# Ipsedo/MusicGAN

Hardware: AMD Instinct MI355X
Metric: spectrogram-images/sec G+D step, 2x128x128 bs64 (higher is better)
Workload: dtype f32

## Files before the change

musicgan_amd/csrc/wino_strip.hip:

```cpp
#include <cstdlib>
#include <type_traits>
#include <utility>

#include "mg_common.h"
#include "pack_kernels.h"
#include "wino_common.h"

namespace {

typedef float f32x2 __attribute__((ext_vector_type(2)));
typedef unsigned u32x2 __attribute__((ext_vector_type(2)));
typedef unsigned u32x4 __attribute__((ext_vector_type(4)));

enum StripKind {
  SK_ACT = 0,
  SK_ACT_POOL_MOUT,
  SK_MB_POOL,
  SK_MASKF,
  SK_UNPOOL,
  SK_BLEND_FWD,
  SK_BLEND_TAN,
  SK_BLEND_BWD,
  SK_PN,
  SK_MB_Y,
};

__device__ __forceinline__ unsigned f2u(float v) { return __builtin_bit_cast(unsigned, v); }
__device__ __forceinline__ int f2i(float v) { return __builtin_bit_cast(int, v); }
__device__ __forceinline__ int clamp01(int v) { return v < 0 ? 0 : (v > 1 ? 1 : v); }
__device__ __forceinline__ float sel_bits(int t, float x, float y) {
  return __builtin_bit_cast(float, (t & f2i(x)) | (~t & f2i(y)));
}

template <class F, int... Is>
__device__ __forceinline__ void sk_static_for_impl(F&& f, std::integer_sequence<int, Is...>) {
  (f(std::integral_constant<int, Is>{}), ...);
}
template <int N, class F>
__device__ __forceinline__ void sk_static_for(F&& f) {
  sk_static_for_impl(f, std::make_integer_sequence<int, N>{});
}
template <int OFF>
__device__ __forceinline__ f32x4 sk_lds128(unsigned addr) {
  f32x4 v;
  asm volatile("ds_read_b128 %0, %1 offset:%2" : "=v"(v) : "v"(addr), "n"(OFF));
  return v;
}
__device__ __forceinline__ void sk_wait() { asm volatile("s_waitcnt lgkmcnt(0)" ::: "memory"); }
__device__ __forceinline__ void sk_tie(f32x4& v) { asm volatile("" : "+v"(v)); }

template <int NIW, int NLDS, int NWAVE, int KIND, bool POOL>
__device__ __forceinline__ void strip_body(const WinoArgs& a, const int ct0, const int wg, const int G) {
  constexpr int kind = KIND;
  constexpr int NTHR = 64 * NWAVE;
  extern __shared__ __attribute__((aligned(16))) float smem[];
  float* Us = smem;
  const int tid = threadIdx.x;
  const int lane = tid & 63, col = lane & 15, rq = lane >> 4;
  const int wave = __builtin_amdgcn_readfirstlane(tid >> 6);
  const int HW = a.H * a.W;
  const int Ht = a.H >> 1, Wt = a.W >> 1;
  const int PP = Ht * Wt;

  {
    const int n4 = a.nchunk * NLDS * 512;
    const f32x4* src = reinterpret_cast<const f32x4*>(a.up);
    f32x4* dst = reinterpret_cast<f32x4*>(Us);
    for (int i = tid; i < n4; i += NTHR) {
      const int ch = i / (NLDS * 512), r = i - ch * (NLDS * 512);
      dst[i] = src[((size_t)ch * a.NT + ct0) * 512 + r];
    }
  }
  __syncthreads();

  const int groups_y = Ht / NWAVE;
  const int nitems = a.N * groups_y * a.blocks_x;
  const int first = mg_xcd_remap(wg, G);
  if (first >= nitems) return;
  const int dbx = G % a.blocks_x, dgy = (G / a.blocks_x) % groups_y, dn = G / (a.blocks_x * groups_y);
  int bx = first % a.blocks_x, gy = (first / a.blocks_x) % groups_y, n0 = first / (a.blocks_x * groups_y);
  int item = first;
  int by = gy * NWAVE + wave;
  auto step = [&](int& item_, int& bx_, int& gy_, int& n_) __attribute__((always_inline)) {
    item_ += G;
    bx_ += dbx;
    const int c1 = bx_ >= a.blocks_x ? 1 : 0;
    bx_ -= c1 * a.blocks_x;
    gy_ += dgy + c1;
    const int c2 = gy_ >= groups_y ? 1 : 0;
    gy_ -= c2 * groups_y;
    n_ += dn + c2;
  };
  auto advance = [&]() __attribute__((always_inline)) {
    step(item, bx, gy, n0);
    by = gy * NWAVE + wave;
  };

  const int lp = ((2 * rq) * HW + 2 * col) * 4;
  unsigned vP, vX;
  int rowoff[4];
  int rowrec[4];
  const float* img_base;
  auto block_geometry = [&]() __attribute__((always_inline)) {
    img_base = a.x + (size_t)n0 * a.Cin * HW;
    const int xoff = bx * 128;
    vP = (unsigned)(lp + xoff);
    vX = col == 0 ? (bx == 0 ? 0x80000000u : vP - 4u) : ((col == 15 && bx != a.blocks_x - 1) ? vP + 8u : 0x80000000u);
#pragma unroll
    for (int r = 0; r < 4; ++r) {
      const int Y = 2 * by - 1 + r;
      rowoff[r] = Y * a.W * 4;
      rowrec[r] = (item < nitems && Y >= 0 && Y < a.H && !(a.TBN & 2)) ? a.Cin * HW * 4 : 0;
    }
  };

  f32x4 acc[16][NIW];
  f32x2 rP[2][4];
  float rX[2][4];
  f32x2 V[2][8];

  auto load_rows = [&](int ch) __attribute__((always_inline)) {
#pragma unroll
    for (int r = 0; r < 4; ++r) {
      const __amdgpu_buffer_rsrc_t rsrc = __builtin_amdgcn_make_buffer_rsrc(const_cast<float*>(img_base), 0, rowrec[r], 0x00020000);
#pragma unroll
      for (int ks = 0; ks < 2; ++ks) {
        const int soff = (ch * WCC + ks) * HW * 4 + rowoff[r];
        rP[ks][r] = __builtin_bit_cast(f32x2, __builtin_amdgcn_raw_buffer_load_b64(rsrc, (int)vP, soff, 0));
        rX[ks][r] = __builtin_bit_cast(float, __builtin_amdgcn_raw_buffer_load_b32(rsrc, (int)vX, soff, 0));
      }
    }
  };

  auto transform_rows = [&]() __attribute__((always_inline)) {
#pragma unroll
    for (int ks = 0; ks < 2; ++ks) {
      f32x2 rE[4];
#pragma unroll
      for (int r = 0; r < 4; ++r) {
        const int old = __builtin_bit_cast(int, rX[ks][r]);
        rE[r][0] = __builtin_bit_cast(float, __builtin_amdgcn_update_dpp(old, __builtin_bit_cast(int, f2i(rP[ks][r][1])), 0x111, 0xf, 0xf, false));
        rE[r][1] = __builtin_bit_cast(float, __builtin_amdgcn_update_dpp(old, __builtin_bit_cast(int, f2i(rP[ks][r][0])), 0x101, 0xf, 0xf, false));
      }
      f32x2 UE[4], UP[4];
      UE[0] = pk_sub(rE[0], rE[2]);  UP[0] = pk_sub(rP[ks][0], rP[ks][2]);
      UE[1] = rE[1] + rE[2];         UP[1] = rP[ks][1] + rP[ks][2];
      UE[2] = pk_sub(rE[2], rE[1]);  UP[2] = pk_sub(rP[ks][2], rP[ks][1]);
      UE[3] = pk_sub(rE[1], rE[3]);  UP[3] = pk_sub(rP[ks][1], rP[ks][3]);
      asm("v_pk_add_f32 %0, %8, %12 op_sel:[0,1] op_sel_hi:[1,0] neg_lo:[0,1] neg_hi:[1,0]\n\t"
          "v_pk_add_f32 %1, %12, %12 op_sel:[0,1] op_sel_hi:[1,0] neg_lo:[0,0] neg_hi:[0,1]\n\t"
          "v_pk_add_f32 %2, %9, %13 op_sel:[0,1] op_sel_hi:[1,0] neg_lo:[0,1] neg_hi:[1,0]\n\t"
          "v_pk_add_f32 %3, %13, %13 op_sel:[0,1] op_sel_hi:[1,0] neg_lo:[0,0] neg_hi:[0,1]\n\t"
          "v_pk_add_f32 %4, %10, %14 op_sel:[0,1] op_sel_hi:[1,0] neg_lo:[0,1] neg_hi:[1,0]\n\t"
          "v_pk_add_f32 %5, %14, %14 op_sel:[0,1] op_sel_hi:[1,0] neg_lo:[0,0] neg_hi:[0,1]\n\t"
          "v_pk_add_f32 %6, %11, %15 op_sel:[0,1] op_sel_hi:[1,0] neg_lo:[0,1] neg_hi:[1,0]\n\t"
          "v_pk_add_f32 %7, %15, %15 op_sel:[0,1] op_sel_hi:[1,0] neg_lo:[0,0] neg_hi:[0,1]\n\t"
          "s_nop 1"
          : "=&v"(V[ks][0]), "=&v"(V[ks][1]), "=&v"(V[ks][2]), "=&v"(V[ks][3]), "=&v"(V[ks][4]), "=&v"(V[ks][5]), "=&v"(V[ks][6]), "=&v"(V[ks][7])
          : "v"(UE[0]), "v"(UE[1]), "v"(UE[2]), "v"(UE[3]), "v"(UP[0]), "v"(UP[1]), "v"(UP[2]), "v"(UP[3]));
    }
  };

  const unsigned us_lane = (unsigned)reinterpret_cast<size_t>(Us + lane * 4);
  auto mfma_chunk = [&](int ch, auto first_) __attribute__((always_inline)) {
    constexpr bool FIRST = decltype(first_)::value;
    const unsigned ub = us_lane + (unsigned)(ch * NLDS) * 8192u;
    f32x4 bv[2][NIW];
    sk_static_for<NIW>([&](auto ni_) __attribute__((always_inline)) {
      constexpr int ni = decltype(ni_)::value;
      bv[0][ni] = sk_lds128<ni * 8192>(ub);
    });
    sk_static_for<8>([&](auto cp_) __attribute__((always_inline)) {
      constexpr int cp = decltype(cp_)::value;
      constexpr int cur = cp & 1, nxt = cur ^ 1;
      sk_wait();
#pragma unroll
      for (int ni = 0; ni < NIW; ++ni) sk_tie(bv[cur][ni]);
      if constexpr (cp + 1 < 8) {
        sk_static_for<NIW>([&](auto ni_) __attribute__((always_inline)) {
          constexpr int ni = decltype(ni_)::value;
          bv[nxt][ni] = sk_lds128<ni * 8192 + (cp + 1) * 1024>(ub);
        });
      }
      __builtin_amdgcn_sched_barrier(0);
#pragma unroll
      for (int ks = 0; ks < 2; ++ks)
#pragma unroll
        for (int par = 0; par < 2; ++par)
#pragma unroll
          for (int ni = 0; ni < NIW; ++ni) {
            const f32x4 c0 = (FIRST && ks == 0) ? f32x4{0.f, 0.f, 0.f, 0.f} : acc[2 * cp + par][ni];
            acc[2 * cp + par][ni] = __builtin_amdgcn_mfma_f32_16x16x4f32(bv[cur][ni][ks * 2 + par], V[ks][cp][par], c0, 0, 0, 0);
          }
      __builtin_amdgcn_sched_barrier(0);
    });
  };

  const bool lrelu = (a.flags & MG_CONV_LRELU) != 0;
  const float slope = a.slope;
  const float slope_eff = lrelu ? slope : 1.0f;
  auto bias4 = [&](int ni) __attribute__((always_inline)) {
    f32x4 b = f32x4{0.f, 0.f, 0.f, 0.f};
    if (a.bias != nullptr) b = *reinterpret_cast<const f32x4*>(a.bias + (ct0 + ni) * 16 + rq * 4);
    return b;
  };
  auto xform = [&](int ni, f32x4 (&r4)[4]) __attribute__((always_inline)) {
    asm volatile("s_nop 7\n\ts_nop 7" : "+v"(acc[0][ni]), "+v"(acc[1][ni]), "+v"(acc[2][ni]), "+v"(acc[3][ni]), "+v"(acc[4][ni]),
                 "+v"(acc[5][ni]), "+v"(acc[6][ni]), "+v"(acc[7][ni]));
    asm volatile("" : "+v"(acc[8][ni]), "+v"(acc[9][ni]), "+v"(acc[10][ni]), "+v"(acc[11][ni]), "+v"(acc[12][ni]), "+v"(acc[13][ni]),
                 "+v"(acc[14][ni]), "+v"(acc[15][ni]));
    constexpr int SL[4] = {0, 2, 3, 1};
    f32x4 s0[4], s1[4];
#pragma unroll
    for (int nu = 0; nu < 4; ++nu) {
      const f32x4 m0 = acc[SL[nu]][ni], m1 = acc[4 + SL[nu]][ni], m2 = acc[8 + SL[nu]][ni], m3 = acc[12 + SL[nu]][ni];
      s0[nu] = (m0 + m1) + m2;
      s1[nu] = pk_sub4(pk_sub4(m1, m2), m3);
    }
    r4[0] = (s0[0] + s0[1]) + s0[2];
    r4[1] = pk_sub4(pk_sub4(s0[1], s0[2]), s0[3]);
    r4[2] = (s1[0] + s1[1]) + s1[2];
    r4[3] = pk_sub4(pk_sub4(s1[1], s1[2]), s1[3]);
  };
  auto activate = [&](int ni, f32x4 (&r4)[4]) __attribute__((always_inline)) {
    const f32x4 b4 = bias4(ni);
#pragma unroll
    for (int q = 0; q < 4; ++q) {
      const f32x4 v = r4[q] + b4;
      const f32x4 w = v * slope_eff;
#pragma unroll
      for (int g = 0; g < 4; ++g) r4[q][g] = fmaxf(v[g], w[g]);
    }
  };
  auto mask_bits = [&](const f32x4 (&r4)[4], int g) __attribute__((always_inline)) {
    const int b0 = clamp01(f2i(r4[0][g])), b1 = clamp01(f2i(r4[1][g])), b2 = clamp01(f2i(r4[2][g])), b3 = clamp01(f2i(r4[3][g]));
    return ((b0 | (b1 << 1)) | (b2 << 2)) | (b3 << 3);
  };
  auto apply_mask_bytes = [&](f32x4 (&r4)[4], const unsigned (&mb)[4]) __attribute__((always_inline)) {
#pragma unroll
    for (int q = 0; q < 4; ++q) {
      const f32x4 os = r4[q] * slope;
#pragma unroll
      for (int g = 0; g < 4; ++g) r4[q][g] = sel_bits(__builtin_amdgcn_sbfe((int)mb[g], q, 1), r4[q][g], os[g]);
    }
  };

  auto acc_fence = [&]() __attribute__((always_inline)) {};
  const int ly = ((rq * 4) * HW + 2 * col) * 4;
  const int lpo = ((rq * 4) * PP + col) * 4;
  using T_ = std::true_type;
  using F_ = std::false_type;

  const int nch = a.nchunk;
  block_geometry();
  load_rows(0);
  transform_rows();
#pragma nounroll
  for (;;) {
    const int ebx = bx, eby = by, en0 = n0;
    load_rows(1);
    mfma_chunk(0, T_{});
    for (int ch = 1; ch + 1 < nch; ++ch) {
      transform_rows();
      load_rows(ch + 1);
      mfma_chunk(ch, F_{});
    }
    transform_rows();
    advance();
    block_geometry();
    load_rows(0);
    mfma_chunk(nch - 1, F_{});
    __builtin_amdgcn_sched_barrier(0);
    acc_fence();
    transform_rows();
    __builtin_amdgcn_sched_barrier(0);

    {
      const int sy = ((2 * eby) * a.W + 32 * ebx) * 4;
      const int sp = (eby * Wt + 16 * ebx) * 4;
      const int yoff = ly, poff = lpo;
      const int TX = ebx * 16 + col;
      const int W4 = a.W * 4;
      auto rs = [&](const void* base, size_t img_elems, int esize) __attribute__((always_inline)) {
        return __builtin_amdgcn_make_buffer_rsrc(const_cast<char*>(reinterpret_cast<const char*>(base)) + (size_t)en0 * img_elems * esize,
                                                 0, (a.TBN & 4) ? 0 : (int)(img_elems * esize), 0x00020000);
      };
      const size_t full = (size_t)a.Cout * HW, pooled_n = (size_t)a.Cout * PP;
      auto store_rows = [&](__amdgpu_buffer_rsrc_t r, const f32x4 (&r4)[4], int ni) __attribute__((always_inline)) {
#pragma unroll
        for (int g4 = 0; g4 < 4; ++g4) {
          const int so = ((ct0 + ni) * 16 + g4) * HW * 4 + sy;
          __builtin_amdgcn_raw_buffer_store_b64(__builtin_bit_cast(u32x2, f32x2{r4[0][g4], r4[1][g4]}), r, yoff, so, 0);
          __builtin_amdgcn_raw_buffer_store_b64(__builtin_bit_cast(u32x2, f32x2{r4[2][g4], r4[3][g4]}), r, yoff, so + W4, 0);
        }
      };
      auto load_rows_f = [&](__amdgpu_buffer_rsrc_t r, f32x4 (&o4)[4], int ni) __attribute__((always_inline)) {
#pragma unroll
        for (int g4 = 0; g4 < 4; ++g4) {
          const int so = ((ct0 + ni) * 16 + g4) * HW * 4 + sy;
          const f32x2 t0 = __builtin_bit_cast(f32x2, __builtin_amdgcn_raw_buffer_load_b64(r, yoff, so, 0));
          const f32x2 t1 = __builtin_bit_cast(f32x2, __builtin_amdgcn_raw_buffer_load_b64(r, yoff, so + W4, 0));
          o4[0][g4] = t0[0]; o4[1][g4] = t0[1]; o4[2][g4] = t1[0]; o4[3][g4] = t1[1];
        }
      };
      auto store_pooled = [&](__amdgpu_buffer_rsrc_t r, const f32x4 (&r4)[4], int ni) __attribute__((always_inline)) {
        const f32x4 pl = ((r4[0] + r4[1]) + (r4[2] + r4[3])) * 0.25f;
#pragma unroll
        for (int g4 = 0; g4 < 4; ++g4)
          __builtin_amdgcn_raw_buffer_store_b32(f2u(pl[g4]), r, poff, ((ct0 + ni) * 16 + g4) * PP * 4 + sp, 0);
      };
      auto load_mask_bytes = [&](__amdgpu_buffer_rsrc_t r, unsigned (&mb)[4], int ni) __attribute__((always_inline)) {
#pragma unroll
        for (int g4 = 0; g4 < 4; ++g4) mb[g4] = __builtin_amdgcn_raw_buffer_load_b8(r, poff >> 2, ((ct0 + ni) * 16 + g4) * PP + (sp >> 2), 0);
      };
      auto store_mask_bytes = [&](__amdgpu_buffer_rsrc_t r, const f32x4 (&r4)[4], int ni) __attribute__((always_inline)) {
#pragma unroll
        for (int g4 = 0; g4 < 4; ++g4)
          __builtin_amdgcn_raw_buffer_store_b8((unsigned char)mask_bits(r4, g4), r, poff >> 2, ((ct0 + ni) * 16 + g4) * PP + (sp >> 2), 0);
      };
      constexpr bool act_on = false;

      if constexpr (kind == SK_ACT_POOL_MOUT) {
        const auto rp = rs(a.p, pooled_n, 4), rm = rs(a.mo, pooled_n, 1);
#pragma unroll
        for (int ni = 0; ni < NIW; ++ni) {
          f32x4 r4[4];
          xform(ni, r4);
          activate(ni, r4);
          store_mask_bytes(rm, r4, ni);
          store_pooled(rp, r4, ni);
        }
      } else if constexpr (kind == SK_MB_POOL) {
        const auto rp = rs(a.p, pooled_n, 4), rm = rs(a.mi, pooled_n, 1);
#pragma unroll
        for (int ni = 0; ni < NIW; ++ni) {
          unsigned mb[4];
          load_mask_bytes(rm, mb, ni);
          f32x4 r4[4];
          xform(ni, r4);
          if (act_on) activate(ni, r4);
          apply_mask_bytes(r4, mb);
          store_pooled(rp, r4, ni);
        }
      } else if constexpr (kind == SK_ACT) {
        const auto ry = rs(a.y, full, 4), rp = rs(a.p, pooled_n, 4);
#pragma unroll
        for (int ni = 0; ni < NIW; ++ni) {
          f32x4 r4[4];
          xform(ni, r4);
          activate(ni, r4);
          store_rows(ry, r4, ni);
          if (POOL) store_pooled(rp, r4, ni);
        }
      } else if constexpr (kind == SK_MASKF) {
        const auto ry = rs(a.y, full, 4), rx = rs(a.aux, full, 4), rp = rs(a.p, pooled_n, 4);
#pragma unroll
        for (int ni = 0; ni < NIW; ++ni) {
          f32x4 ax[4];
          load_rows_f(rx, ax, ni);
          f32x4 r4[4];
          xform(ni, r4);
          if (act_on) activate(ni, r4);
#pragma unroll
          for (int q = 0; q < 4; ++q) {
            const f32x4 os = r4[q] * slope;
#pragma unroll
            for (int g4 = 0; g4 < 4; ++g4) r4[q][g4] = ax[q][g4] > 0.f ? r4[q][g4] : os[g4];
          }
          store_rows(ry, r4, ni);
          if (POOL) store_pooled(rp, r4, ni);
        }
      } else if constexpr (kind == SK_UNPOOL) {
        const auto ry = rs(a.y, 4 * full, 4), rm = rs(a.aux, full, 1);
        const int uoff = yoff >> 2, su = sy >> 2;
        const int y2off = ((rq * 4) * 4 * HW + 4 * col) * 4;
        const int sy2 = ((4 * eby) * (2 * a.W) + 64 * ebx) * 4;
        const float qh = 0.25f, ql = 0.25f * slope;
#pragma unroll
        for (int ni = 0; ni < NIW; ++ni) {
          unsigned mw[4][2];
#pragma unroll
          for (int g4 = 0; g4 < 4; ++g4)
#pragma unroll
            for (int i = 0; i < 2; ++i)
              mw[g4][i] = __builtin_amdgcn_raw_buffer_load_b16(rm, uoff, ((ct0 + ni) * 16 + g4) * HW + i * a.W + su, 0);
          f32x4 r4[4];
          xform(ni, r4);
#pragma unroll
          for (int g4 = 0; g4 < 4; ++g4)
#pragma unroll
            for (int i = 0; i < 2; ++i) {
              const float vh[2] = {r4[2 * i][g4] * qh, r4[2 * i + 1][g4] * qh}, vl[2] = {r4[2 * i][g4] * ql, r4[2 * i + 1][g4] * ql};
#pragma unroll
              for (int r = 0; r < 2; ++r) {
                f32x4 o;
#pragma unroll
                for (int e = 0; e < 2; ++e)
#pragma unroll
                  for (int jj = 0; jj < 2; ++jj)
                    o[e * 2 + jj] = sel_bits(__builtin_amdgcn_sbfe((int)mw[g4][i], 8 * e + 2 * r + jj, 1), vh[e], vl[e]);
                __builtin_amdgcn_raw_buffer_store_b128(__builtin_bit_cast(u32x4, o), ry, y2off,
                                                       (((ct0 + ni) * 16 + g4) * 4 * HW + (2 * i + r) * 2 * a.W) * 4 + sy2, 0);
                asm volatile("s_nop 1" : "+v"(o) : : "memory");
              }
            }
        }
      } else if constexpr (kind == SK_BLEND_FWD || kind == SK_BLEND_TAN) {
        const auto ry = rs(a.y, full, 4), ro = rs(a.other, full, 4);
        const auto rm = rs(kind == SK_BLEND_FWD ? static_cast<const void*>(a.mo) : static_cast<const void*>(a.mi), pooled_n, 1);
        const float bca = a.coef[0], bcb = a.coef[1];
#pragma unroll
        for (int ni = 0; ni < NIW; ++ni) {
          f32x4 o4[4];
          load_rows_f(ro, o4, ni);
          unsigned mb[4] = {15u, 15u, 15u, 15u};
          if (kind == SK_BLEND_TAN) load_mask_bytes(rm, mb, ni);
          f32x4 r4[4];
          xform(ni, r4);
          if (kind == SK_BLEND_FWD || act_on) activate(ni, r4);
          if (kind == SK_BLEND_TAN) apply_mask_bytes(r4, mb);
          else store_mask_bytes(rm, r4, ni);
#pragma unroll
          for (int q = 0; q < 4; ++q) r4[q] = bca * r4[q] + bcb * o4[q];
          store_rows(ry, r4, ni);
        }
      } else if constexpr (kind == SK_BLEND_BWD) {
        const auto ry = rs(a.y, full, 4), rp = rs(a.p, full, 4), ro = rs(a.other, full, 4), rm = rs(a.mi, pooled_n, 1);
        const float ca = a.coef[0], cb = a.coef[1];
#pragma unroll
        for (int ni = 0; ni < NIW; ++ni) {
          f32x4 o4[4];
          load_rows_f(ro, o4, ni);
          unsigned mb[4];
          load_mask_bytes(rm, mb, ni);
          f32x4 r4[4], ra[4], rb[4];
          xform(ni, r4);
#pragma unroll
          for (int q = 0; q < 4; ++q) {
            ra[q] = ca * r4[q];
            rb[q] = cb * r4[q];
            const f32x4 bs = rb[q] * slope;
#pragma unroll
            for (int g4 = 0; g4 < 4; ++g4) rb[q][g4] = o4[q][g4] > 0.f ? rb[q][g4] : bs[g4];
          }
          apply_mask_bytes(ra, mb);
          store_rows(ry, ra, ni);
          store_rows(rp, rb, ni);
        }
      } else if constexpr (kind == SK_MB_Y) {
        const auto ry = rs(a.y, full, 4), rm = rs(a.mi, pooled_n, 1);
#pragma unroll
        for (int ni = 0; ni < NIW; ++ni) {
          unsigned mb[4];
          load_mask_bytes(rm, mb, ni);
          f32x4 r4[4];
          xform(ni, r4);
          apply_mask_bytes(r4, mb);
          store_rows(ry, r4, ni);
        }
      } else {
        const auto rp = rs(a.p, full, 4);
        f32x4 o[NIW][4];
#pragma unroll
        for (int ni = 0; ni < NIW; ++ni) {
          xform(ni, o[ni]);
          activate(ni, o[ni]);
        }
        float rnv[4];
#pragma unroll
        for (int q = 0; q < 4; ++q) {
          float t = 0.f;
#pragma unroll
          for (int ni = 0; ni < NIW; ++ni) {
            float tn = 0.f;
#pragma unroll
            for (int g4 = 0; g4 < 4; ++g4) tn += o[ni][q][g4] * o[ni][q][g4];
            tn += __shfl_xor(tn, 16);
            tn += __shfl_xor(tn, 32);
            t += tn;
          }
          rnv[q] = 1.0f / sqrtf(t / (float)a.Cout + PN_EPS);
        }
#pragma unroll
        for (int ni = 0; ni < NIW; ++ni) {
#pragma unroll
          for (int q = 0; q < 4; ++q) o[ni][q] = o[ni][q] * rnv[q];
          store_rows(rp, o[ni], ni);
        }
        if (rq == 0 && a.rn != nullptr) {
          float* rn = a.rn + ((size_t)en0 * a.H + 2 * eby) * a.W + 2 * TX;
          *reinterpret_cast<float2*>(rn) = make_float2(rnv[0], rnv[1]);
          *reinterpret_cast<float2*>(rn + a.W) = make_float2(rnv[2], rnv[3]);
        }
      }
    }
    if (item >= nitems) break;
  }
}

template <int NIW, int NWAVE, int KIND, bool POOL>
__global__ void __launch_bounds__(64 * NWAVE, (NIW == 1 && KIND != SK_UNPOOL && KIND != SK_PN) ? 3 : 1) wino3x3_strip(const WinoArgs a) {
  const int g_full = a.TBW, g_pad = a.TBH, nrows = a.lgTBW;
  const int row = ((int)blockIdx.x < (nrows - (g_pad ? 1 : 0)) * g_full) ? (int)blockIdx.x / g_full : nrows - 1;
  const int wg = (int)blockIdx.x - row * g_full;
  if (NIW == 2 && g_pad != 0 && row == nrows - 1) strip_body<1, NIW, NWAVE, KIND, POOL>(a, row * NIW, wg, g_pad);
  else strip_body<NIW, NIW, NWAVE, KIND, POOL>(a, row * NIW, wg, g_full);
}

template <int NIW, int NWAVE, int KIND, bool POOL>
int launch_strip(const WinoArgs& a, dim3 grid, hipStream_t s) {
  const size_t lds = (size_t)a.nchunk * NIW * 2048 * sizeof(float);
  static MgPerDevice once;
  const void* fn = reinterpret_cast<const void*>(&wino3x3_strip<NIW, NWAVE, KIND, POOL>);
  if (mg_first_use_on_device(once)) (void)hipFuncSetAttribute(fn, hipFuncAttributeMaxDynamicSharedMemorySize, 160 * 1024);
  static struct { int dev; size_t lds; int v; } occ[8];
  static int nocc = 0;
  int per_cu = 0;
  const int dev = mg_current_device();
  for (int i = 0; i < nocc && i < 8; ++i)
    if (occ[i].dev == dev && occ[i].lds == lds) per_cu = occ[i].v;
  if (per_cu == 0) {
    if (hipOccupancyMaxActiveBlocksPerMultiprocessor(&per_cu, fn, 64 * NWAVE, lds) != hipSuccess || per_cu < 1) per_cu = 1;
    if (per_cu > 16 / NWAVE) per_cu = 16 / NWAVE;
    if (nocc < 8) { occ[nocc].dev = dev; occ[nocc].lds = lds; occ[nocc].v = per_cu; ++nocc; }
  }
  {
    const char* e = getenv("MG_WINO_STRIP_WGS");
    if (e != nullptr && atoi(e) >= 1) per_cu = atoi(e);
  }
  const int rows = (int)grid.y, nt = a.Cout / 16;
  const bool has_pad = NIW == 2 && (nt & 1) != 0 && rows > 1;
  const int total = per_cu * mg_cu_count();
  static const double pad_w = getenv("MG_WINO_STRIP_PADW") ? atof(getenv("MG_WINO_STRIP_PADW")) : 0.7;
  int g_pad = 0, g_full;
  if (has_pad) {
    g_pad = (int)(total * pad_w / ((rows - 1) + pad_w)) & ~7;
    if (g_pad < 8) g_pad = 8;
    g_full = ((total - g_pad) / (rows - 1)) & ~7;
  } else {
    g_full = (total / rows) & ~7;
  }
  if (g_full < 8) g_full = 8;
  const int nitems = a.N * (a.blocks_y / NWAVE) * a.blocks_x;
  if (g_full > nitems) g_full = nitems;
  if (g_pad > nitems) g_pad = nitems;
  WinoArgs b = a;
  b.TBW = g_full; b.TBH = g_pad; b.lgTBW = rows;
  grid = dim3((unsigned)((rows - (g_pad ? 1 : 0)) * g_full + g_pad), 1, 1);
  hipLaunchKernelGGL((wino3x3_strip<NIW, NWAVE, KIND, POOL>), grid, dim3(64 * NWAVE), lds, s, b);
  MG_CHECK_LAUNCH("mg_wino3x3 (strip)");
  return MG_OK;
}

template <int NIW, int NWAVE>
int launch_strip_kind(const WinoArgs& a, int kind, dim3 grid, hipStream_t s) {
  const bool pool = (a.flags & MG_CONV_POOL_OUT) != 0;
  switch (kind) {
    case SK_ACT: return pool ? launch_strip<NIW, NWAVE, SK_ACT, true>(a, grid, s) : launch_strip<NIW, NWAVE, SK_ACT, false>(a, grid, s);
    case SK_ACT_POOL_MOUT: return launch_strip<NIW, NWAVE, SK_ACT_POOL_MOUT, true>(a, grid, s);
    case SK_MB_POOL: return launch_strip<NIW, NWAVE, SK_MB_POOL, true>(a, grid, s);
    case SK_MASKF: return pool ? launch_strip<NIW, NWAVE, SK_MASKF, true>(a, grid, s) : launch_strip<NIW, NWAVE, SK_MASKF, false>(a, grid, s);
    case SK_UNPOOL: return launch_strip<NIW, NWAVE, SK_UNPOOL, false>(a, grid, s);
    case SK_BLEND_FWD: return launch_strip<NIW, NWAVE, SK_BLEND_FWD, false>(a, grid, s);
    case SK_BLEND_TAN: return launch_strip<NIW, NWAVE, SK_BLEND_TAN, false>(a, grid, s);
    case SK_BLEND_BWD: return launch_strip<NIW, NWAVE, SK_BLEND_BWD, false>(a, grid, s);
    case SK_MB_Y: return launch_strip<NIW, NWAVE, SK_MB_Y, false>(a, grid, s);
    default:
      if constexpr (NIW <= 2) return launch_strip<NIW, NWAVE, SK_PN, false>(a, grid, s);
      mg_set_error("mg_wino3x3 (strip): PixelNorm with three out-channel tiles");
      return MG_EINVAL;
  }
}

long long strip_min_blocks() {
  static const long long v = getenv("MG_WINO_STRIP_MIN_BLOCKS") ? atoll(getenv("MG_WINO_STRIP_MIN_BLOCKS")) : 2048;
  return v;
}

int strip_plan(const WinoArgs& a, bool pn, bool force) {
  const int nt = a.Cout / 16;
  const long long blocks = (long long)a.N * (a.H / 2) * (a.W / 32);
  int niw = 0;
  niw = (force || blocks >= strip_min_blocks()) ? (nt == 1 ? 1 : 2) : 0;
  if (niw == 2 && (size_t)(a.Cin / WCC) * 2 * 8192 > 160 * 1024) niw = 1;
  if (pn) niw = nt <= 2 ? (niw ? nt : 0) : 0;
  const char* e = getenv("MG_WINO_STRIP_NIW");
  if (e != nullptr && !pn && niw != 0) {
    const int v = atoi(e);
    if (v == 1 || (v == 2 && nt >= 2) || (v == 3 && nt == 3)) niw = v;
  }
  return niw;
}

int strip_kind(const WinoArgs& a) {
  if (a.flags & MG_CONV_PIXNORM) return SK_PN;
  if (a.flags & MG_CONV_UNPOOL) return SK_UNPOOL;
  if (a.flags & WF_BLEND_BWD) return SK_BLEND_BWD;
  if (a.flags & WF_BLEND) return (a.flags & MG_CONV_MASK_BYTES) ? SK_BLEND_TAN : SK_BLEND_FWD;
  if (a.flags & MG_CONV_MASK_AUX) return (a.flags & MG_CONV_MASK_BYTES) ? ((a.flags & MG_CONV_POOL_OUT) ? SK_MB_POOL : SK_MB_Y) : SK_MASKF;
  return (a.flags & MG_CONV_MASK_OUT) ? SK_ACT_POOL_MOUT : SK_ACT;
}

}

bool mgi_wino_strip_takes(const WinoArgs& a, bool pn) {
  const char* e = getenv("MG_WINO_STRIP");
  if (e != nullptr && atoi(e) == 0) return false;
  const int nt = a.Cout / 16;
  if ((a.Cin % 16) != 0 || (a.Cout % 16) != 0 || nt > 10 || (a.W % 32) != 0 || ((a.H / 2) % 8) != 0 || (a.H % 2) != 0) return false;
  if (pn && (nt > 2 || a.y != nullptr)) return false;
  if ((a.flags & (MG_CONV_MASK_AUX | MG_CONV_UNPOOL | WF_BLEND_BWD)) && a.bias != nullptr) return false;
  if ((long long)a.Cout * a.H * a.W * 16 >= (1ll << 31) || (long long)a.Cin * a.H * a.W * 4 >= (1ll << 31)) return false;
  const int niw = strip_plan(a, pn, e != nullptr && atoi(e) > 1);
  return niw != 0 && (size_t)(a.Cin / WCC) * niw * 8192 <= 160 * 1024;
}

int mgi_wino_strip_run(WinoArgs& a, hipStream_t s) {
  const int nt = a.Cout / 16;
  a.nchunk = a.Cin / WCC;
  a.NT = pack_wino_nt_padded(a.Cout);
  a.TBW = 16; a.TBH = 1; a.TBN = 1; a.lgTBW = 4; a.lgTBH = 0;
  {
    const char* e = getenv("MG_WINO_STRIP_ABLATE");
    if (e != nullptr) a.TBN |= atoi(e) & 6;
  }
  a.blocks_x = a.W / 32; a.blocks_y = a.H / 2; a.blocks_n = a.N;
  const int kind = strip_kind(a);
  const char* e = getenv("MG_WINO_STRIP");
  const int niw = strip_plan(a, kind == SK_PN, e != nullptr && atoi(e) > 1);
  dim3 grid(1, mg_cdiv(nt, niw));
  switch (niw) {
    case 1: return launch_strip_kind<1, 8>(a, kind, grid, s);
    case 2: return launch_strip_kind<2, 8>(a, kind, grid, s);
    default: return launch_strip_kind<3, 4>(a, kind, grid, s);
  }
}
```

Before: 5589.

## Prefetch epilogue mask loads before next-block geometry and pipeline blend-bwd row loads

Moves the buffer descriptors and helper lambdas ahead of the main loop body so that the mask-byte loads for the blend-backward and unpool epilogues are issued right after the last chunk's transform, before the next block's first loads and final MFMA chunk. Their latency can then overlap the remaining MFMA work instead of stalling the epilogue. The blend-backward epilogue also double-buffers the 'other' row loads, fetching the next sub-tile's rows while the current one is being processed. The cost is extra live registers for the prefetched masks and buffered rows, which may raise register pressure and lower occupancy.

```diff
diff --git a/musicgan_amd/csrc/wino_strip.hip b/musicgan_amd/csrc/wino_strip.hip
--- a/musicgan_amd/csrc/wino_strip.hip
+++ b/musicgan_amd/csrc/wino_strip.hip
@@ -258,6 +258,49 @@
 #pragma nounroll
   for (;;) {
     const int ebx = bx, eby = by, en0 = n0;
+    const int sy = ((2 * eby) * a.W + 32 * ebx) * 4;
+    const int sp = (eby * Wt + 16 * ebx) * 4;
+    const int yoff = ly, poff = lpo;
+    const int TX = ebx * 16 + col;
+    const int W4 = a.W * 4;
+    auto rs = [&](const void* base, size_t img_elems, int esize) __attribute__((always_inline)) {
+      return __builtin_amdgcn_make_buffer_rsrc(const_cast<char*>(reinterpret_cast<const char*>(base)) + (size_t)en0 * img_elems * esize,
+                                               0, (a.TBN & 4) ? 0 : (int)(img_elems * esize), 0x00020000);
+    };
+    const size_t full = (size_t)a.Cout * HW, pooled_n = (size_t)a.Cout * PP;
+    auto load_rows_f = [&](__amdgpu_buffer_rsrc_t r, f32x4 (&o4)[4], int ni) __attribute__((always_inline)) {
+#pragma unroll
+      for (int g4 = 0; g4 < 4; ++g4) {
+        const int so = ((ct0 + ni) * 16 + g4) * HW * 4 + sy;
+        const f32x2 t0 = __builtin_bit_cast(f32x2, __builtin_amdgcn_raw_buffer_load_b64(r, yoff, so, 0));
+        const f32x2 t1 = __builtin_bit_cast(f32x2, __builtin_amdgcn_raw_buffer_load_b64(r, yoff, so + W4, 0));
+        o4[0][g4] = t0[0]; o4[1][g4] = t0[1]; o4[2][g4] = t1[0]; o4[3][g4] = t1[1];
+      }
+    };
+    auto load_mask_bytes = [&](__amdgpu_buffer_rsrc_t r, unsigned (&mb)[4], int ni) __attribute__((always_inline)) {
+#pragma unroll
+      for (int g4 = 0; g4 < 4; ++g4) mb[g4] = __builtin_amdgcn_raw_buffer_load_b8(r, poff >> 2, ((ct0 + ni) * 16 + g4) * PP + (sp >> 2), 0);
+    };
+    unsigned emb[NIW][4];
+    unsigned emw[NIW][4][2];
+    auto epilogue_requests = [&]() __attribute__((always_inline)) {
+      if constexpr (kind == SK_BLEND_BWD) {
+        const auto rm = rs(a.mi, pooled_n, 1);
+#pragma unroll
+        for (int ni = 0; ni < NIW; ++ni) load_mask_bytes(rm, emb[ni], ni);
+      }
+      if constexpr (kind == SK_UNPOOL) {
+        const auto rm = rs(a.aux, full, 1);
+        const int uoff = yoff >> 2, su = sy >> 2;
+#pragma unroll
+        for (int ni = 0; ni < NIW; ++ni)
+#pragma unroll
+          for (int g4 = 0; g4 < 4; ++g4)
+#pragma unroll
+            for (int i = 0; i < 2; ++i)
+              emw[ni][g4][i] = __builtin_amdgcn_raw_buffer_load_b16(rm, uoff, ((ct0 + ni) * 16 + g4) * HW + i * a.W + su, 0);
+      }
+    };
     load_rows(1);
     mfma_chunk(0, T_{});
     for (int ch = 1; ch + 1 < nch; ++ch) {
@@ -266,6 +309,7 @@
       mfma_chunk(ch, F_{});
     }
     transform_rows();
+    epilogue_requests();
     advance();
     block_geometry();
     load_rows(0);
@@ -276,16 +320,6 @@
     __builtin_amdgcn_sched_barrier(0);
 
     {
-      const int sy = ((2 * eby) * a.W + 32 * ebx) * 4;
-      const int sp = (eby * Wt + 16 * ebx) * 4;
-      const int yoff = ly, poff = lpo;
-      const int TX = ebx * 16 + col;
-      const int W4 = a.W * 4;
-      auto rs = [&](const void* base, size_t img_elems, int esize) __attribute__((always_inline)) {
-        return __builtin_amdgcn_make_buffer_rsrc(const_cast<char*>(reinterpret_cast<const char*>(base)) + (size_t)en0 * img_elems * esize,
-                                                 0, (a.TBN & 4) ? 0 : (int)(img_elems * esize), 0x00020000);
-      };
-      const size_t full = (size_t)a.Cout * HW, pooled_n = (size_t)a.Cout * PP;
       auto store_rows = [&](__amdgpu_buffer_rsrc_t r, const f32x4 (&r4)[4], int ni) __attribute__((always_inline)) {
 #pragma unroll
         for (int g4 = 0; g4 < 4; ++g4) {
@@ -294,24 +328,11 @@
           __builtin_amdgcn_raw_buffer_store_b64(__builtin_bit_cast(u32x2, f32x2{r4[2][g4], r4[3][g4]}), r, yoff, so + W4, 0);
         }
       };
-      auto load_rows_f = [&](__amdgpu_buffer_rsrc_t r, f32x4 (&o4)[4], int ni) __attribute__((always_inline)) {
-#pragma unroll
-        for (int g4 = 0; g4 < 4; ++g4) {
-          const int so = ((ct0 + ni) * 16 + g4) * HW * 4 + sy;
-          const f32x2 t0 = __builtin_bit_cast(f32x2, __builtin_amdgcn_raw_buffer_load_b64(r, yoff, so, 0));
-          const f32x2 t1 = __builtin_bit_cast(f32x2, __builtin_amdgcn_raw_buffer_load_b64(r, yoff, so + W4, 0));
-          o4[0][g4] = t0[0]; o4[1][g4] = t0[1]; o4[2][g4] = t1[0]; o4[3][g4] = t1[1];
-        }
-      };
       auto store_pooled = [&](__amdgpu_buffer_rsrc_t r, const f32x4 (&r4)[4], int ni) __attribute__((always_inline)) {
         const f32x4 pl = ((r4[0] + r4[1]) + (r4[2] + r4[3])) * 0.25f;
 #pragma unroll
         for (int g4 = 0; g4 < 4; ++g4)
           __builtin_amdgcn_raw_buffer_store_b32(f2u(pl[g4]), r, poff, ((ct0 + ni) * 16 + g4) * PP * 4 + sp, 0);
-      };
-      auto load_mask_bytes = [&](__amdgpu_buffer_rsrc_t r, unsigned (&mb)[4], int ni) __attribute__((always_inline)) {
-#pragma unroll
-        for (int g4 = 0; g4 < 4; ++g4) mb[g4] = __builtin_amdgcn_raw_buffer_load_b8(r, poff >> 2, ((ct0 + ni) * 16 + g4) * PP + (sp >> 2), 0);
       };
       auto store_mask_bytes = [&](__amdgpu_buffer_rsrc_t r, const f32x4 (&r4)[4], int ni) __attribute__((always_inline)) {
 #pragma unroll
@@ -371,19 +392,13 @@
           if (POOL) store_pooled(rp, r4, ni);
         }
       } else if constexpr (kind == SK_UNPOOL) {
-        const auto ry = rs(a.y, 4 * full, 4), rm = rs(a.aux, full, 1);
-        const int uoff = yoff >> 2, su = sy >> 2;
+        const auto ry = rs(a.y, 4 * full, 4);
         const int y2off = ((rq * 4) * 4 * HW + 4 * col) * 4;
         const int sy2 = ((4 * eby) * (2 * a.W) + 64 * ebx) * 4;
         const float qh = 0.25f, ql = 0.25f * slope;
 #pragma unroll
         for (int ni = 0; ni < NIW; ++ni) {
-          unsigned mw[4][2];
-#pragma unroll
-          for (int g4 = 0; g4 < 4; ++g4)
-#pragma unroll
-            for (int i = 0; i < 2; ++i)
-              mw[g4][i] = __builtin_amdgcn_raw_buffer_load_b16(rm, uoff, ((ct0 + ni) * 16 + g4) * HW + i * a.W + su, 0);
+          const unsigned (&mw)[4][2] = emw[ni];
           f32x4 r4[4];
           xform(ni, r4);
 #pragma unroll
@@ -425,14 +440,14 @@
           store_rows(ry, r4, ni);
         }
       } else if constexpr (kind == SK_BLEND_BWD) {
-        const auto ry = rs(a.y, full, 4), rp = rs(a.p, full, 4), ro = rs(a.other, full, 4), rm = rs(a.mi, pooled_n, 1);
+        const auto ry = rs(a.y, full, 4), rp = rs(a.p, full, 4), ro = rs(a.other, full, 4);
         const float ca = a.coef[0], cb = a.coef[1];
-#pragma unroll
-        for (int ni = 0; ni < NIW; ++ni) {
-          f32x4 o4[4];
-          load_rows_f(ro, o4, ni);
-          unsigned mb[4];
-          load_mask_bytes(rm, mb, ni);
+        f32x4 ob[NIW][4];
+        load_rows_f(ro, ob[0], 0);
+#pragma unroll
+        for (int ni = 0; ni < NIW; ++ni) {
+          if (ni + 1 < NIW) load_rows_f(ro, ob[ni + 1 < NIW ? ni + 1 : 0], ni + 1);
+          const f32x4 (&o4)[4] = ob[ni];
           f32x4 r4[4], ra[4], rb[4];
           xform(ni, r4);
 #pragma unroll
@@ -443,7 +458,7 @@
 #pragma unroll
             for (int g4 = 0; g4 < 4; ++g4) rb[q][g4] = o4[q][g4] > 0.f ? rb[q][g4] : bs[g4];
           }
-          apply_mask_bytes(ra, mb);
+          apply_mask_bytes(ra, emb[ni]);
           store_rows(ry, ra, ni);
           store_rows(rp, rb, ni);
         }
```

Result: no change. 5603, median of 6 (+0.3%).
